# Advanced-Vision-and-Learning-Lab/sparse-view-3dgs-pack

Hardware: AMD Instinct MI355X
Metric: train-step views/s (fwd+bwd) @1M Gaussians 1080p (higher is better)
Workload: dtype f32

## Files before the change

sparse-view-3dgs-pack_amd/csrc/gs_regionbin.hip:

```cpp
#include "gs_common.h"
#include "gs_tilecull.h"

#define RB_THREADS 1024
#define RB_WAVES (RB_THREADS / 64)
#define RB_TILES (RG_TILES * RG_TILES)

__global__ void __launch_bounds__(GS_BLOCK) region_prepare_kernel(GeomHeader* hdr, uint32_t* __restrict__ region_count,
                                                                   int regions, uint32_t P) {
  const int i = blockIdx.x * GS_BLOCK + threadIdx.x;
  if (i < regions) region_count[(size_t)i * RG_COUNT_STRIDE] = 0u;
  if (i == 0) {
    hdr->num_rendered = 0u;
    hdr->overflow = 0u;
    hdr->trunc_failed = 0u;
    hdr->zero = 0u;
    hdr->P = P;
    hdr->sort_n = 0u;
    hdr->n_ordered = 0u;
    hdr->region_mode = 1u;
    hdr->pad[HDR_SIDE_CURSOR] = 0u;
  }
}

__global__ void __launch_bounds__(RB_THREADS) region_bin_kernel(GeomHeader* hdr, const Splat* __restrict__ splat,
                                                                 const uint32_t* __restrict__ region_count,
                                                                 const uint2* __restrict__ region_bucket, uint32_t region_cap,
                                                                 int rg_x, int grid_x, int grid_y,
                                                                 const float* __restrict__ depth_limit,
                                                                 uint2* __restrict__ ranges, uint32_t* __restrict__ point_list,
                                                                 uint32_t capacity, uint32_t n_pad_max) {
  extern __shared__ unsigned long long s_key[];
  __shared__ uint32_t s_wcnt[RB_WAVES][RB_TILES];
  __shared__ uint32_t s_off[RB_TILES + 1];
  __shared__ uint32_t s_base;
  __shared__ float s_lim[RB_TILES];
  const int tid = threadIdx.x, lane = tid & 63, wid = tid >> 6;
  const int r = blockIdx.x, rx = r % rg_x, ry = r / rg_x;
  const uint32_t cnt_raw = region_count[(size_t)r * RG_COUNT_STRIDE];
  const uint32_t n = min(min(cnt_raw, region_cap), n_pad_max);
  if (tid == 0) {
    atomicMax(&hdr->zero, cnt_raw);
    if (cnt_raw > n) hdr->overflow = 1u;
  }
  if (tid < RB_TILES) {
    const int ty = ry * RG_TILES + (tid >> 2), tx = rx * RG_TILES + (tid & 3);
    s_lim[tid] = (depth_limit && ty < grid_y && tx < grid_x) ? depth_limit[ty * grid_x + tx] : __builtin_inff();
  }
  uint32_t n_pad = 64;
  while (n_pad < n) n_pad <<= 1;
  const uint2* bucket = region_bucket + (size_t)r * region_cap;
  for (uint32_t i = tid; i < n_pad; i += RB_THREADS) {
    unsigned long long k = ~0ull;
    if (i < n) {
      const uint2 e = bucket[i];
      k = ((unsigned long long)e.x << 32) | (unsigned long long)e.y;
    }
    s_key[i] = k;
  }
  __syncthreads();
  auto step = [&](uint32_t k, uint32_t j) {
    for (uint32_t i = tid; i < (n_pad >> 1); i += RB_THREADS) {
      const uint32_t lo = ((i & ~(j - 1u)) << 1) | (i & (j - 1u));
      const uint32_t hi = lo | j;
      const unsigned long long a = s_key[lo], b = s_key[hi];
      const bool up = (lo & k) == 0u;
      if ((a > b) == up) {
        s_key[lo] = b;
        s_key[hi] = a;
      }
    }
  };
  for (uint32_t k = 2; k <= n_pad; k <<= 1) {
    uint32_t j = k >> 1;
    for (; j > 64; j >>= 1) {
      step(k, j);
      __syncthreads();
    }
    for (; j > 0; j >>= 1) {
      step(k, j);
      __builtin_amdgcn_fence(__ATOMIC_RELEASE, "wavefront");
      __builtin_amdgcn_wave_barrier();
      __builtin_amdgcn_fence(__ATOMIC_ACQUIRE, "wavefront");
    }
    if (k >= 128u || k == n_pad) __syncthreads();
  }
  for (uint32_t e = tid; e < n; e += RB_THREADS) {
    const uint32_t id = (uint32_t)s_key[e];
    const float4* rec = reinterpret_cast<const float4*>(&splat[id]);
    const float4 ra = rec[0], rc = rec[1];
    const uint4 tail = reinterpret_cast<const uint4*>(rec)[3];
    const TileCull tc = tilecull_setup(1, ra.x, ra.y, rc.x, rc.y, rc.z, rc.w);
    const uint32_t rminx = tail.x & 0xFFFFu, rminy = tail.x >> 16, rmaxx = tail.y & 0xFFFFu, rmaxy = tail.y >> 16;
    uint32_t mask = 0;
#pragma unroll
    for (uint32_t k = 0; k < RG_TILES; k++) {
      const uint32_t ty = (uint32_t)ry * RG_TILES + k;
      if (ty < rminy || ty >= rmaxy) continue;
      uint32_t tx0;
      const uint32_t nt = tilecull_row_span(tc, ty, rminx, rmaxx, tx0);
      if (nt == 0) continue;
      const int c0 = max((int)tx0 - rx * RG_TILES, 0), c1 = min((int)(tx0 + nt) - rx * RG_TILES, RG_TILES);
      if (c1 > c0) mask |= (((1u << (c1 - c0)) - 1u) << c0) << (4u * k);
    }
    if (depth_limit) {
#pragma unroll
      for (uint32_t t = 0; t < RB_TILES; t++)
        if (depth_beyond_limit(ra.z, s_lim[t])) mask &= ~(1u << t);
    }
    s_key[e] = ((unsigned long long)mask << 32) | (unsigned long long)id;
  }
  __syncthreads();
  const uint32_t per_wave = ((n + RB_WAVES * 64 - 1) / (RB_WAVES * 64)) * 64;
  const uint32_t w_lo = min((uint32_t)wid * per_wave, n), w_hi = min(w_lo + per_wave, n);
  uint32_t my_cnt = 0;
  for (uint32_t e0 = w_lo; e0 < w_hi; e0 += 64) {
    const uint32_t e = e0 + lane;
    const uint32_t m = e < w_hi ? (uint32_t)(s_key[e] >> 32) : 0u;
#pragma unroll
    for (uint32_t t = 0; t < RB_TILES; t++) {
      const uint32_t c = (uint32_t)__popcll(__ballot((m >> t) & 1u));
      if (lane == (int)t) my_cnt += c;
    }
  }
  if (lane < RB_TILES) s_wcnt[wid][lane] = my_cnt;
  __syncthreads();
  if (tid < RB_TILES) {
    uint32_t run = 0;
#pragma unroll
    for (int w = 0; w < RB_WAVES; w++) {
      const uint32_t c = s_wcnt[w][tid];
      s_wcnt[w][tid] = run;
      run += c;
    }
    s_off[tid + 1] = run;
  }
  __syncthreads();
  if (tid == 0) {
    uint32_t run = 0;
    s_off[0] = 0;
    for (int t = 0; t < RB_TILES; t++) {
      const uint32_t c = s_off[t + 1];
      s_off[t] = run;
      run += c;
    }
    s_off[RB_TILES] = run;
    uint32_t base = 0xFFFFFFFFu;
    if (run) {
      const uint32_t at = atomicAdd(&hdr->num_rendered, run);
      if ((unsigned long long)at + run <= (unsigned long long)capacity) base = at;
      else hdr->overflow = 1u;
    } else {
      base = 0u;
    }
    s_base = base;
  }
  __syncthreads();
  const uint32_t base = s_base;
  if (tid < RB_TILES) {
    const int ty = ry * RG_TILES + (tid >> 2), tx = rx * RG_TILES + (tid & 3);
    if (ty < grid_y && tx < grid_x) {
      const uint32_t b = base + s_off[tid], c = s_off[tid + 1] - s_off[tid];
      ranges[ty * grid_x + tx] = (base == 0xFFFFFFFFu || c == 0u) ? make_uint2(0u, 0u) : make_uint2(b, b + c);
    }
  }
  if (base == 0xFFFFFFFFu) return;
  uint32_t run = 0;
  const unsigned long long lt_mask = lane == 0 ? 0ull : (~0ull >> (64 - lane));
  for (uint32_t e0 = w_lo; e0 < w_hi; e0 += 64) {
    const uint32_t e = e0 + lane;
    const unsigned long long k = e < w_hi ? s_key[e] : 0ull;
    const uint32_t m = (uint32_t)(k >> 32), id = (uint32_t)k;
#pragma unroll
    for (uint32_t t = 0; t < RB_TILES; t++) {
      const unsigned long long b = __ballot((m >> t) & 1u);
      const uint32_t before = (uint32_t)__shfl((int)run, (int)t, 64);
      if ((m >> t) & 1u) point_list[base + s_off[t] + s_wcnt[wid][t] + before + (uint32_t)__popcll(b & lt_mask)] = id;
      if (lane == (int)t) run += (uint32_t)__popcll(b);
    }
  }
}

__global__ void __launch_bounds__(GS_BLOCK) export_keys_region_kernel(const uint2* __restrict__ ranges,
                                                                      const uint32_t* __restrict__ point_list,
                                                                      const Splat* __restrict__ splat,
                                                                      uint64_t* __restrict__ keys_sorted) {
  const uint2 r = ranges[blockIdx.x];
  for (uint32_t i = r.x + threadIdx.x; i < r.y; i += GS_BLOCK)
    keys_sorted[i] = ((uint64_t)blockIdx.x << 32) | (uint64_t)__float_as_uint(splat[point_list[i]].depth);
}

int launch_region_prepare(const GeomView& g, uint32_t* region_count, int regions, uint32_t P, hipStream_t s) {
  hipLaunchKernelGGL(region_prepare_kernel, dim3((regions + GS_BLOCK - 1) / GS_BLOCK > 0 ? (regions + GS_BLOCK - 1) / GS_BLOCK : 1),
                     dim3(GS_BLOCK), 0, s, g.hdr, region_count, regions, P);
  return 0;
}

int launch_region_bin(const GeomView& g, const uint32_t* region_count, const uint2* region_bucket, uint32_t region_cap, int rg_x,
                      int rg_y, int grid_x, int grid_y, const float* tile_depth_limit, uint2* ranges, uint32_t* point_list,
                      int64_t capacity, hipStream_t s) {
  uint32_t n_pad = 1024;
  while (n_pad < region_cap && n_pad < RG_MAX_ENTRIES) n_pad <<= 1;
  const size_t lds = (size_t)n_pad * sizeof(unsigned long long);
  static_assert(RG_MAX_ENTRIES * sizeof(unsigned long long) <= 160 * 1024, "a region's sort must fit gfx950's 160 KB of LDS");
  static size_t lds_allowed[64] = {};
  int dev = 0;
  if (hipGetDevice(&dev) != hipSuccess || dev < 0 || dev >= 64) dev = -1;
  if (dev < 0 || lds > lds_allowed[dev]) {
    hipError_t e = hipFuncSetAttribute((const void*)region_bin_kernel, hipFuncAttributeMaxDynamicSharedMemorySize, (int)lds);
    if (e != hipSuccess) return (int)e;
    if (dev >= 0) lds_allowed[dev] = lds;
  }
  const uint32_t cap32 = capacity > 0xFFFFFFFFll ? 0xFFFFFFFFu : (capacity < 0 ? 0u : (uint32_t)capacity);
  hipLaunchKernelGGL(region_bin_kernel, dim3(rg_x * rg_y), dim3(RB_THREADS), lds, s, g.hdr, g.splat, region_count, region_bucket,
                     region_cap, rg_x, grid_x, grid_y, tile_depth_limit, ranges, point_list, cap32, n_pad);
  const hipError_t le = hipGetLastError();
  return le == hipSuccess ? 0 : (int)le;
}

int launch_export_keys_region(const uint2* ranges, const uint32_t* point_list, const Splat* splat, int T, uint64_t* keys_sorted,
                              hipStream_t s) {
  hipLaunchKernelGGL(export_keys_region_kernel, dim3(T), dim3(GS_BLOCK), 0, s, ranges, point_list, splat, keys_sorted);
  return 0;
}
```

Before: 1182.

## Use mirrored bitonic sort without padding and batch splat gathers in region binning

Replaces the padded bitonic sort with a one-directional variant that compares each element against its mirrored partner on the first step of every merge stage. Compares whose partner lies beyond n are skipped, so sentinel padding writes and wasted compare-swaps on padded slots go away. The per-element splat fetch is restructured to issue four gathers before computing tile masks, which raises memory-level parallelism at the cost of more registers. It also adds optional compile-time phase clocks for profiling, which are off by default.

```diff
diff --git a/sparse-view-3dgs-pack_amd/csrc/gs_regionbin.hip b/sparse-view-3dgs-pack_amd/csrc/gs_regionbin.hip
--- a/sparse-view-3dgs-pack_amd/csrc/gs_regionbin.hip
+++ b/sparse-view-3dgs-pack_amd/csrc/gs_regionbin.hip
@@ -4,6 +4,22 @@
 #define RB_THREADS 1024
 #define RB_WAVES (RB_THREADS / 64)
 #define RB_TILES (RG_TILES * RG_TILES)
+#define RB_GATHER 4
+
+#ifdef RB_PHASE_CLOCKS
+#define RB_CLOCK_REGIONS 4096
+__device__ unsigned long long rb_phase_clock[RB_CLOCK_REGIONS][8];
+#define RB_CLOCK(slot)                                                                                   \
+  do {                                                                                                   \
+    if (threadIdx.x == 0 && blockIdx.x < RB_CLOCK_REGIONS) rb_phase_clock[blockIdx.x][slot] = wall_clock64(); \
+  } while (0)
+extern "C" int rbdbg_read_phase_clocks(unsigned long long* host_out, int regions) {
+  if (regions < 0 || regions > RB_CLOCK_REGIONS) return -1;
+  return (int)hipMemcpyFromSymbol(host_out, HIP_SYMBOL(rb_phase_clock), sizeof(unsigned long long) * 8 * (size_t)regions);
+}
+#else
+#define RB_CLOCK(slot) do {} while (0)
+#endif
 
 __global__ void __launch_bounds__(GS_BLOCK) region_prepare_kernel(GeomHeader* hdr, uint32_t* __restrict__ region_count,
                                                                    int regions, uint32_t P) {
@@ -36,6 +52,7 @@
   __shared__ float s_lim[RB_TILES];
   const int tid = threadIdx.x, lane = tid & 63, wid = tid >> 6;
   const int r = blockIdx.x, rx = r % rg_x, ry = r / rg_x;
+  RB_CLOCK(0);
   const uint32_t cnt_raw = region_count[(size_t)r * RG_COUNT_STRIDE];
   const uint32_t n = min(min(cnt_raw, region_cap), n_pad_max);
   if (tid == 0) {
@@ -49,67 +66,87 @@
   uint32_t n_pad = 64;
   while (n_pad < n) n_pad <<= 1;
   const uint2* bucket = region_bucket + (size_t)r * region_cap;
-  for (uint32_t i = tid; i < n_pad; i += RB_THREADS) {
-    unsigned long long k = ~0ull;
-    if (i < n) {
-      const uint2 e = bucket[i];
-      k = ((unsigned long long)e.x << 32) | (unsigned long long)e.y;
-    }
-    s_key[i] = k;
-  }
-  __syncthreads();
-  auto step = [&](uint32_t k, uint32_t j) {
+  for (uint32_t i = tid; i < n; i += RB_THREADS) {
+    const uint2 e = bucket[i];
+    s_key[i] = ((unsigned long long)e.x << 32) | (unsigned long long)e.y;
+  }
+  __syncthreads();
+  RB_CLOCK(1);
+  auto step = [&](uint32_t j, bool mirror) {
+    const uint32_t flip = mirror ? 2u * j - 1u : j;
     for (uint32_t i = tid; i < (n_pad >> 1); i += RB_THREADS) {
       const uint32_t lo = ((i & ~(j - 1u)) << 1) | (i & (j - 1u));
-      const uint32_t hi = lo | j;
-      const unsigned long long a = s_key[lo], b = s_key[hi];
-      const bool up = (lo & k) == 0u;
-      if ((a > b) == up) {
-        s_key[lo] = b;
-        s_key[hi] = a;
+      const uint32_t hi = lo ^ flip;
+      if (hi < n) {
+        const unsigned long long a = s_key[lo], b = s_key[hi];
+        if (a > b) {
+          s_key[lo] = b;
+          s_key[hi] = a;
+        }
       }
     }
   };
   for (uint32_t k = 2; k <= n_pad; k <<= 1) {
+    bool mirror = true;
     uint32_t j = k >> 1;
     for (; j > 64; j >>= 1) {
-      step(k, j);
+      step(j, mirror);
+      mirror = false;
       __syncthreads();
     }
     for (; j > 0; j >>= 1) {
-      step(k, j);
+      step(j, mirror);
+      mirror = false;
       __builtin_amdgcn_fence(__ATOMIC_RELEASE, "wavefront");
       __builtin_amdgcn_wave_barrier();
       __builtin_amdgcn_fence(__ATOMIC_ACQUIRE, "wavefront");
     }
     if (k >= 128u || k == n_pad) __syncthreads();
   }
-  for (uint32_t e = tid; e < n; e += RB_THREADS) {
-    const uint32_t id = (uint32_t)s_key[e];
-    const float4* rec = reinterpret_cast<const float4*>(&splat[id]);
-    const float4 ra = rec[0], rc = rec[1];
-    const uint4 tail = reinterpret_cast<const uint4*>(rec)[3];
-    const TileCull tc = tilecull_setup(1, ra.x, ra.y, rc.x, rc.y, rc.z, rc.w);
-    const uint32_t rminx = tail.x & 0xFFFFu, rminy = tail.x >> 16, rmaxx = tail.y & 0xFFFFu, rmaxy = tail.y >> 16;
-    uint32_t mask = 0;
-#pragma unroll
-    for (uint32_t k = 0; k < RG_TILES; k++) {
-      const uint32_t ty = (uint32_t)ry * RG_TILES + k;
-      if (ty < rminy || ty >= rmaxy) continue;
-      uint32_t tx0;
-      const uint32_t nt = tilecull_row_span(tc, ty, rminx, rmaxx, tx0);
-      if (nt == 0) continue;
-      const int c0 = max((int)tx0 - rx * RG_TILES, 0), c1 = min((int)(tx0 + nt) - rx * RG_TILES, RG_TILES);
-      if (c1 > c0) mask |= (((1u << (c1 - c0)) - 1u) << c0) << (4u * k);
-    }
-    if (depth_limit) {
-#pragma unroll
-      for (uint32_t t = 0; t < RB_TILES; t++)
-        if (depth_beyond_limit(ra.z, s_lim[t])) mask &= ~(1u << t);
-    }
-    s_key[e] = ((unsigned long long)mask << 32) | (unsigned long long)id;
-  }
-  __syncthreads();
+  RB_CLOCK(2);
+  for (uint32_t e0 = tid; e0 < n; e0 += RB_GATHER * RB_THREADS) {
+    uint32_t id[RB_GATHER];
+    float4 ra[RB_GATHER], rc[RB_GATHER];
+    uint2 rect[RB_GATHER];
+#pragma unroll
+    for (int g = 0; g < RB_GATHER; g++) {
+      const uint32_t e = e0 + g * RB_THREADS;
+      id[g] = (uint32_t)s_key[e < n ? e : e0];
+    }
+#pragma unroll
+    for (int g = 0; g < RB_GATHER; g++) {
+      const float4* rec = reinterpret_cast<const float4*>(&splat[id[g]]);
+      ra[g] = rec[0];
+      rc[g] = rec[1];
+      rect[g] = reinterpret_cast<const uint2*>(rec)[6];
+    }
+#pragma unroll
+    for (int g = 0; g < RB_GATHER; g++) {
+      const uint32_t e = e0 + g * RB_THREADS;
+      if (e >= n) break;
+      const TileCull tc = tilecull_setup(1, ra[g].x, ra[g].y, rc[g].x, rc[g].y, rc[g].z, rc[g].w);
+      const uint32_t rminx = rect[g].x & 0xFFFFu, rminy = rect[g].x >> 16, rmaxx = rect[g].y & 0xFFFFu, rmaxy = rect[g].y >> 16;
+      uint32_t mask = 0;
+#pragma unroll
+      for (uint32_t k = 0; k < RG_TILES; k++) {
+        const uint32_t ty = (uint32_t)ry * RG_TILES + k;
+        if (ty < rminy || ty >= rmaxy) continue;
+        uint32_t tx0;
+        const uint32_t nt = tilecull_row_span(tc, ty, rminx, rmaxx, tx0);
+        if (nt == 0) continue;
+        const int c0 = max((int)tx0 - rx * RG_TILES, 0), c1 = min((int)(tx0 + nt) - rx * RG_TILES, RG_TILES);
+        if (c1 > c0) mask |= (((1u << (c1 - c0)) - 1u) << c0) << (4u * k);
+      }
+      if (depth_limit) {
+#pragma unroll
+        for (uint32_t t = 0; t < RB_TILES; t++)
+          if (depth_beyond_limit(ra[g].z, s_lim[t])) mask &= ~(1u << t);
+      }
+      s_key[e] = ((unsigned long long)mask << 32) | (unsigned long long)id[g];
+    }
+  }
+  __syncthreads();
+  RB_CLOCK(3);
   const uint32_t per_wave = ((n + RB_WAVES * 64 - 1) / (RB_WAVES * 64)) * 64;
   const uint32_t w_lo = min((uint32_t)wid * per_wave, n), w_hi = min(w_lo + per_wave, n);
   uint32_t my_cnt = 0;
@@ -135,6 +172,7 @@
     s_off[tid + 1] = run;
   }
   __syncthreads();
+  RB_CLOCK(4);
   if (tid == 0) {
     uint32_t run = 0;
     s_off[0] = 0;
@@ -155,6 +193,7 @@
     s_base = base;
   }
   __syncthreads();
+  RB_CLOCK(5);
   const uint32_t base = s_base;
   if (tid < RB_TILES) {
     const int ty = ry * RG_TILES + (tid >> 2), tx = rx * RG_TILES + (tid & 3);
@@ -178,6 +217,11 @@
       if (lane == (int)t) run += (uint32_t)__popcll(b);
     }
   }
+#ifdef RB_PHASE_CLOCKS
+  __syncthreads();
+  RB_CLOCK(6);
+  if (tid == 0 && r < RB_CLOCK_REGIONS) rb_phase_clock[r][7] = n;
+#endif
 }
 
 __global__ void __launch_bounds__(GS_BLOCK) export_keys_region_kernel(const uint2* __restrict__ ranges,
```

Result: slower. 1162 (-1.6%).
